# GAP-LAB-CUHK-SZ/RfDNet

Hardware: AMD Instinct MI355X
Metric: scenes/sec end-to-end reconstruction (ScanNet, 64^3 MISE) (higher is better)
Workload: dtype f32 (point ops, MLPs); f16x3 split MFMA with f32 accumulate (decoder, fp32-class)

## Files before the change

### include/rfd_pointnet2.h

```cpp
#ifndef RFD_POINTNET2_H
#define RFD_POINTNET2_H

#ifdef __cplusplus
extern "C" {
#endif

int furthest_point_sampling_kernel_wrapper(int b, int n, int m,
                                           const float *dataset, float *temp,
                                           int *idxs, void *stream);

int gather_points_kernel_wrapper(int b, int c, int n, int npoints,
                                 const float *points, const int *idx,
                                 float *out, void *stream);

int gather_points_grad_kernel_wrapper(int b, int c, int n, int npoints,
                                      const float *grad_out, const int *idx,
                                      float *grad_points, void *stream);

int query_ball_point_kernel_wrapper(int b, int n, int m, float radius,
                                    int nsample, const float *new_xyz,
                                    const float *xyz, int *idx, void *stream);

int group_points_kernel_wrapper(int b, int c, int n, int npoints, int nsample,
                                const float *points, const int *idx,
                                float *out, void *stream);

int group_points_grad_kernel_wrapper(int b, int c, int n, int npoints,
                                     int nsample, const float *grad_out,
                                     const int *idx, float *grad_points,
                                     void *stream);

int three_nn_kernel_wrapper(int b, int n, int m, const float *unknown,
                            const float *known, float *dist2, int *idx,
                            void *stream);

int three_interpolate_kernel_wrapper(int b, int c, int m, int n,
                                     const float *points, const int *idx,
                                     const float *weight, float *out,
                                     void *stream);

int three_interpolate_grad_kernel_wrapper(int b, int c, int n, int m,
                                          const float *grad_out,
                                          const int *idx, const float *weight,
                                          float *grad_points, void *stream);


int rfd_group_concat(int b, int c, int n, int m, int nsample, float radius,
                     int normalize, int use_xyz, const float *xyz,
                     const float *new_xyz, const float *features,
                     const int *idx, float *out, float *grouped_xyz_out,
                     void *stream);

int rfd_furthest_point_sampling_gather(int b, int n, int m,
                                       const float *dataset, float *temp,
                                       int *idxs, float *new_xyz,
                                       void *stream);

const char *rfd_last_error_string(void);
enum {
  RFD_STATUS_FPS_ABORT = 1,
  RFD_STATUS_DECODER_RANGE = 2,
  RFD_STATUS_GEMM_RANGE = 4
};
int rfd_device_status(void);
int rfd_stream_status(void *stream);
int rfd_stream_status_snapshot(void *stream, unsigned *host_word);
int rfd_release_stream(void *stream);
int rfd_fps_set_timeout_ms(int ms);
int rfd_fps_set_geometry(int points_per_thread);
int rfd_fps_test_phantom_units(int n);
int rfd_test_hold_cus(int leave_free_cus, const unsigned *release_flag, int max_ms, void *stream);
const char *rfd_build_arch(void);

int rfd_three_interpolate_cat(int b, int c, int cs, int m, int n, const float *points, const int *idx,
                              const float *dist2, const float *skip, float *out, void *stream);
int rfd_mlp_cols(int B, int N, int n_layers, const int *widths, const float *const *wt, const float *const *bias,
                 const int *relu, const float *x, float *y, void *stream);

int rfd_sa_fused(int b, int n, int m, int nsample, int c_feat, float radius, int normalize_xyz,
                 const float *xyz, const float *new_xyz, const float *features, const int *idx,
                 int c1, int c2, int c3, const float *w1, const float *b1, const float *w2,
                 const float *b2, const float *w3, const float *b3, float *out, void *stream);

#ifdef __cplusplus
}
#endif
#endif
```

### rfdnet_amd/_lib.py

```python
import ctypes as C
import os

_HERE = os.path.dirname(os.path.abspath(__file__))
LIB_PATH = os.environ.get("RFD_HIP_LIB") or os.path.join(_HERE, "lib", "librfd_hip.so")

_f = C.c_void_p
_i = C.c_int
_fl = C.c_float
_sz = C.c_size_t
_d = C.c_double

OPTIONAL = "optional"
ABI = {
    "furthest_point_sampling_kernel_wrapper": (_i, [_i, _i, _i, _f, _f, _f, _f]),
    "gather_points_kernel_wrapper": (_i, [_i, _i, _i, _i, _f, _f, _f, _f]),
    "gather_points_grad_kernel_wrapper": (_i, [_i, _i, _i, _i, _f, _f, _f, _f]),
    "query_ball_point_kernel_wrapper": (_i, [_i, _i, _i, _fl, _i, _f, _f, _f, _f]),
    "group_points_kernel_wrapper": (_i, [_i, _i, _i, _i, _i, _f, _f, _f, _f]),
    "group_points_grad_kernel_wrapper": (_i, [_i, _i, _i, _i, _i, _f, _f, _f, _f]),
    "three_nn_kernel_wrapper": (_i, [_i, _i, _i, _f, _f, _f, _f, _f]),
    "three_interpolate_kernel_wrapper": (_i, [_i, _i, _i, _i, _f, _f, _f, _f, _f]),
    "three_interpolate_grad_kernel_wrapper": (_i, [_i, _i, _i, _i, _f, _f, _f, _f, _f]),
    "rfd_group_concat": (_i, [_i, _i, _i, _i, _i, _fl, _i, _i, _f, _f, _f, _f, _f, _f, _f]),
    "rfd_furthest_point_sampling_gather": (_i, [_i, _i, _i, _f, _f, _f, _f, _f]),
    "rfd_chamfer_forward": (_i, [_i, _i, _f, _i, _f, _f, _f, _f, _f, _f]),
    "rfd_chamfer_backward": (_i, [_i, _i, _f, _i, _f, _f, _f, _f, _f, _f, _f, _f]),
    "rfd_sa_fused": (_i, [_i, _i, _i, _i, _i, _fl, _i, _f, _f, _f, _f, _i, _i, _i, _f, _f, _f, _f, _f, _f, _f, _f]),
    "rfd_occ_pack_weights": (_i, [_f, _f, C.POINTER(C.c_int), _i, _f, _f]),
    "rfd_occ_decode": (_i, [_i, _f, _f, _f, _f, _f, _f, _f, _fl, _f, _i, _f]),
    "rfd_occ_pack_weights_w8": (_i, [_f, _f, C.POINTER(C.c_int), _i, _f, _f]),
    "rfd_occ_decode_w8": (_i, [_i, _f, _f, _f, _f, _f, _f, _f, _fl, _f, _i, _f]),
    "rfd_occ_decode_scatter_w8": (_i, [_i, _f, _f, _f, _f, _f, _f, _f, _fl, _f, _f, _f, C.c_longlong, _i, _f]),
    "rfd_occ_chunk_range": (_i, [_i, _i, _i, C.POINTER(C.c_int), C.POINTER(C.c_int)]),
    "rfd_occ_chunk_range_capped": (_i, [_i, _i, _i, _i, C.POINTER(C.c_int), C.POINTER(C.c_int), C.POINTER(C.c_int)]),
    "rfd_occ_set_launch_shape": (_i, [_i, _i, _i]),
    "rfd_occ_set_tail_tiles": (_i, [_i]),
    "rfd_occ_normals_w8": (_i, [_i, _f, _f, _f, _i, _f, _f, C.POINTER(C.c_int), _f, _f, _f, _f, _f, _i, _f]),
    "rfd_refine_sample": (_i, [_i, _i, _f, _f, _f, _f, _f, _f, _f, _f, _f]),
    "rfd_refine_face_backward": (_i, [_i, _i, _f, _f, _f, _f, _f, _f, _f, _f, _fl, _f, _f]),
    "rfd_refine_vertex_step": (_i, [_i, _f, _f, _i, _f, _f, _f, _f, _f]),
    "rfd_refine_dirichlet": (_i, [_i, C.c_ulonglong, _i, _f, _f]),
    "rfd_fps_set_timeout_ms": (_i, [_i]),
    "rfd_fps_set_geometry": (_i, [_i]),
    "rfd_test_hold_cus": (_i, [_i, _f, _i, _f], OPTIONAL),
    "rfd_fps_test_phantom_units": (_i, [_i], OPTIONAL),
    "rfd_make_grid_points": (_i, [_i, _fl, _fl, _fl, _f, _i, _f]),
    "rfd_mise_init": (_i, [_i, _i, _i, _f, _f, _f]),
    "rfd_mise_count": (_i, [_i, _i, _i, _f, _f, _f]),
    "rfd_mise_collect": (_i, [_i, _i, _i, _f, _f, _f, _fl, _f, _f, _f]),
    "rfd_mise_scatter": (_i, [_i, _i, _i, _f, _f, _f, _f, _f, _f, _f]),
    "rfd_mise_subdivide": (_i, [_i, _i, _i, C.c_double, _f, _f, _f, _f]),
    "rfd_mise_subdivide_active": (_i, [_i, _i, _i, C.c_double, _f, _f, _f, _f, _f]),
    "rfd_mise_subdivide_dirty": (_i, [_i, _i, _i, C.c_double, _f, _f, _f, _f, C.c_longlong, _f, _f, _f, _f, _i, _f]),
    "rfd_mise_to_dense": (_i, [_i, _i, _i, _f, _f, _f]),
    "rfd_points_in_boxes": (_i, [_i, _i, _i, _i, _f, _f, _f, _f]),
    "rfd_nms3d": (_i, [_i, _i, C.c_double, _i, _i, _f, _f, _f, _f, _f, _f]),
    "rfd_gemm_pack_w": (_i, [_i, _i, _i, _f, _f, _f]),
    "rfd_gemm_f16x3": (_i, [_i, _i, _i, _f, _i, _f, _f, _i, _f, _f, _i, _f, _i, _i, _i, _i, _i, _f, _i, _f]),
    "rfd_mc_classify": (_i, [_i, _i, _fl, C.c_double, _f, _f, _f, _f, _f]),
    "rfd_mc_emit_affine": (_i, [_i, _i, _fl, C.c_double, _f, _f, _f, _f, _f, _f, _f, C.c_double, C.c_double, _f]),
    "rfd_mc_blocks": (_i, [_i]),
    "rfd_occ_fold_rows": (_i, [_i, _i, _i, _f, _f, _f, _f, _f, _f, _f, _i, _f, _f]),
    "rfd_rows3_rotate_z": (_i, [_i, _i, _f, _f, _f, _f]),
    "rfd_rows3_affine": (_i, [_i, _i, _f, _f, _f, _f]),
    "rfd_mlp_cols": (_i, [_i, _i, _i, _f, _f, _f, _f, _f, _f, _f]),
    "rfd_three_interpolate_cat": (_i, [_i, _i, _i, _i, _i, _f, _f, _f, _f, _f, _f]),
    "rfd_chain_pack_n": (_i, [_i, _i, _f, _f, _f, _i, _i, _i, _f, _f]),
    "rfd_chain_pool_n": (_i, [_i, _i, _i, _i, _i, _f, _i, _f, _f, _f, _f, _f, _i, _i, _i, _i, _i, _f, _f]),
    "rfd_head_pack": (_i, [_f, _f, _f, _i, _i, _i, _f, _f]),
    "rfd_head_scores": (_i, [_i, _i, _f, _i, _f, _f, _f, _f, _f, _f, _i, _i, _i, _i, _i, _f, _f]),
    "rfd_pos_embed": (_i, [_i, _i, _i, _f, _i, _f, _f, _i, _f, _f, _i, _f, _i, _i, _f]),
    "rfd_pos_embed_frag": (_i, [_i, _i, _i, _f, _i, _f, _f, _i, _f, _f, _i, _f, C.c_long, _i, _f]),
    "rfd_rows_to_frag": (_i, [_i, _i, _f, _i, _i, _i, _f, C.c_long, _f]),
    "rfd_frag_to_rows": (_i, [_i, _i, _f, C.c_long, _i, _f, _i, _f]),
    "rfd_gemm_f16x3_frag": (_i, [_i, _i, _i, _f, C.c_long, _f, _f, C.c_long, _f, _f, _i, _i, _i, _i, _f, _i, _f]),
    "rfd_box3d_iou": (_i, [_i, _i, _i, _f, _f, _f, _f, _f]),
    "rfd_ap_match": (_i, [_i, _i, _i, _i, _i, _f, _f, _f, _f, _f, _f, _f, _f]),
    "rfd_latent_prep": (_i, [_i, _i, _f, _f, _f, _f, _f, _f]),
    "rfd_latent_stage": (_i, [_i, _i, _i, _f, _f, _f, _f, _f, _f, _f, _f, _f]),
    "rfd_latent_head": (_i, [_i, _i, _f, _f, _f, _f, _f, _f, _f, _f, _f]),
    "rfd_bce_logits_rowsum": (_i, [_i, _i, _f, _i, _f, _i, _f, _f]),
    "rfd_voxel_iou": (_i, [_i, _i, _f, _i, _fl, _f, _f, _f, _f]),
    "rfd_vote_loss_partial": (_i, [_i, _i, _i, _i, _f, _f, _f, _f, _f, _f, _f]),
    "rfd_proposal_loss_partial": (_i, [_i, _i, _i, _i, _i, _i, _f, _f, _f, _f, _f, _f, _f, _f, C.POINTER(C.c_int), _f, _i, _f, _f,
                                       _f, _f, _f, _f, _f, _f, _f, _f, _i, _f, _f]),
    "rfd_detection_loss_finish": (_i, [_i, _i, _i, _f, _f, _f]),
    "rfd_mask_loss_partial": (_i, [_i, _i, _f, _f, _i, _f, _f, _f, _f]),
    "rfd_mask_loss_finish": (_i, [_i, _i, _fl, _f, _f, _f]),
    "rfd_fit_pose_run": (_i, [_i, _i, _i, _i, _i, _i, C.c_double, C.c_double, _f, _f, _f, _f, _f, _f, _f, _f, _f, _f, _f, _f,
                              _f, _f]),
    "rfd_raster_project": (_i, [_i, _i, _i, _f, _f, C.POINTER(C.c_double), C.c_double, _f, _f, _f, _f]),
    "rfd_raster_triangles": (_i, [_i, _i, _i, _i, _i, _i, _f, _f, _f, _f, _f, _f]),
    "rfd_raster_shade": (_i, [_i, _i, _i, _i, _i, _f, _f, _f, _f, _f, C.POINTER(C.c_double), _f, _f, _f, _f, _f]),
    "rfd_decimate_vertex_keys": (_i, [_i, _i, _i, _i, _f, _f, _f, _f, _f, _f]),
    "rfd_decimate_face_remap": (_i, [_i, _i, _i, _f, _f, _f, _f, _f, _f, _f, _f, _f]),
    "rfd_decimate_parity": (_i, [_i, _i, _i, _f, _f, _f, _f, _f, _f, _f]),
# ... 253 lines not shown
```

### rfdnet_amd/csrc/common.h

```cpp
#pragma once
#include <hip/hip_runtime.h>
#include <stdint.h>
#include <stdio.h>
#include <atomic>
#include "../../include/rfd_pointnet2.h"

#define RFD_API extern "C" __attribute__((visibility("default")))

void rfd_set_error(const char *where, hipError_t e);

#define RFD_CHECK(expr)                        \
  do {                                         \
    hipError_t _e = (expr);                    \
    if (_e != hipSuccess) {                    \
      rfd_set_error(#expr, _e);                \
      return (int)_e;                          \
    }                                          \
  } while (0)

#define RFD_CHECK_LAUNCH()                     \
  do {                                         \
    hipError_t _e = hipGetLastError();         \
    if (_e != hipSuccess) {                    \
      rfd_set_error(__func__, _e);             \
      return (int)_e;                          \
    }                                          \
  } while (0)

static inline int rfd_invalid(const char *msg) {
  const hipError_t e = hipErrorInvalidValue;
  rfd_set_error(msg, e);
  return (int)e;
}

constexpr int RFD_ZEROS_FLOATS = 16384;
constexpr int RFD_STATUS_SLOTS = 64;
constexpr int RFD_FPS_TIMEOUT_MS_DEFAULT = 500;
constexpr int FPS_MAX_WG = 256;
constexpr int FPS_REGION_HEAD = 8;
constexpr int FPS_REGION_GRANULES = FPS_REGION_HEAD + FPS_MAX_WG * 2 * 5;
constexpr int FPS_SHARED_RING = 16;
constexpr int FPS_REGIONS = RFD_STATUS_SLOTS + FPS_SHARED_RING;
constexpr int RFD_CLAIM_SLOTS = 1024;
struct RfdWorkspace {
  unsigned long long *fps_slots;
  unsigned *status;
  std::atomic<void *> status_owner[RFD_STATUS_SLOTS];
  float *zeros;
  unsigned *claim;
  std::atomic<unsigned> claim_seq;
  std::atomic<unsigned> ring_pos;
  int num_cu;
  int wall_clock_khz;
  std::atomic<int> fps_timeout_ms;
  std::atomic<int> fps_force_ppt;
  std::atomic<int> fps_test_phantom;
};
int rfd_get_workspace(RfdWorkspace **ws);
#define RFD_WORKSPACE(ws)                      \
  RfdWorkspace *ws;                            \
  do {                                         \
    int _rc = rfd_get_workspace(&ws);          \
    if (_rc) return _rc;                       \
  } while (0)
int rfd_status_slot(RfdWorkspace *ws, hipStream_t stream);
static inline unsigned *rfd_status_word(RfdWorkspace *ws, hipStream_t stream) {
  return ws->status + rfd_status_slot(ws, stream);
}
static inline unsigned *rfd_claim_pair(RfdWorkspace *ws, hipStream_t stream) {
  const int slot = rfd_status_slot(ws, stream);
  if (slot > 0) return ws->claim + 2 * slot;
  return ws->claim + 2 * (RFD_STATUS_SLOTS + ws->claim_seq.fetch_add(1, std::memory_order_relaxed) %
                                                 (RFD_CLAIM_SLOTS - RFD_STATUS_SLOTS));
}
static inline unsigned long long *rfd_fps_region(RfdWorkspace *ws, hipStream_t stream) {
  const int slot = rfd_status_slot(ws, stream);
  const unsigned r = slot > 0 ? (unsigned)slot
                              : RFD_STATUS_SLOTS + ws->ring_pos.fetch_add(1, std::memory_order_relaxed) % FPS_SHARED_RING;
  return ws->fps_slots + (size_t)r * FPS_REGION_GRANULES;
}

__device__ __forceinline__ float sumsq3(float a, float b, float c) {
  float t = b * b;
  t = __builtin_fmaf(a, a, t);
  t = __builtin_fmaf(c, c, t);
  return t;
}

__device__ __forceinline__ void atomic_max_float(float *p, float v) {
  if (v >= 0.f) atomicMax(reinterpret_cast<int *>(p), __float_as_int(v + 0.f));
  else atomicMin(reinterpret_cast<unsigned *>(p), __float_as_uint(v));
}

static inline int ceil_div(int a, int b) { return (a + b - 1) / b; }

static inline int ref_opt_n_threads(int work_size) {
  const int pow_2 = (int)(log((double)work_size) / log(2.0));
  int v = 1 << pow_2;
  if (v > 512) v = 512;
  if (v < 1) v = 1;
  return v;
}
```

### rfdnet_amd/csrc/runtime.hip

```cpp
#include "common.h"

#include <stdlib.h>

#include <mutex>
#include <string>

namespace {
thread_local std::string g_last_error;
std::mutex g_ws_mutex;
RfdWorkspace *g_ws[64] = {nullptr};
}

void rfd_set_error(const char *where, hipError_t e) {
  g_last_error = std::string(where) + ": " + hipGetErrorString(e);
}

int rfd_get_workspace(RfdWorkspace **out) {
  int dev = 0;
  RFD_CHECK(hipGetDevice(&dev));
  if (dev < 0 || dev >= 64) {
    rfd_set_error("rfd_get_workspace: device index", hipErrorInvalidDevice);
    return (int)hipErrorInvalidDevice;
  }
  std::lock_guard<std::mutex> lk(g_ws_mutex);
  if (!g_ws[dev]) {
    RfdWorkspace *w = new RfdWorkspace();
    RFD_CHECK(hipMalloc((void **)&w->fps_slots,
                        sizeof(unsigned long long) * (size_t)FPS_REGIONS * FPS_REGION_GRANULES));
    RFD_CHECK(hipMalloc((void **)&w->status, sizeof(unsigned) * RFD_STATUS_SLOTS));
    RFD_CHECK(hipMemset(w->status, 0, sizeof(unsigned) * RFD_STATUS_SLOTS));
    for (int i = 0; i < RFD_STATUS_SLOTS; ++i) w->status_owner[i].store(nullptr);
    RFD_CHECK(hipMalloc((void **)&w->zeros, sizeof(float) * RFD_ZEROS_FLOATS));
    RFD_CHECK(hipMemset(w->zeros, 0, sizeof(float) * RFD_ZEROS_FLOATS));
    RFD_CHECK(hipMalloc((void **)&w->claim, sizeof(unsigned) * 2 * RFD_CLAIM_SLOTS));
    RFD_CHECK(hipMemset(w->claim, 0, sizeof(unsigned) * 2 * RFD_CLAIM_SLOTS));
    w->claim_seq.store(0);
    w->ring_pos.store(0);
    w->num_cu = 0;
    (void)hipDeviceGetAttribute(&w->num_cu, hipDeviceAttributeMultiprocessorCount, dev);
    w->wall_clock_khz = 0;
    (void)hipDeviceGetAttribute(&w->wall_clock_khz, hipDeviceAttributeWallClockRate, dev);
    if (w->wall_clock_khz <= 0) w->wall_clock_khz = 100000;
    const char *to = getenv("RFD_FPS_TIMEOUT_MS");
    const int to_ms = to ? atoi(to) : 0;
    w->fps_timeout_ms.store(to_ms > 0 ? to_ms : RFD_FPS_TIMEOUT_MS_DEFAULT);
    w->fps_force_ppt.store(0);
    w->fps_test_phantom.store(0);
    g_ws[dev] = w;
  }
  *out = g_ws[dev];
  return 0;
}

RFD_API const char *rfd_last_error_string(void) { return g_last_error.c_str(); }

int rfd_status_slot(RfdWorkspace *ws, hipStream_t stream) {
  void *key = (void *)stream;
  if (!key) return 0;
  for (int i = 1; i < RFD_STATUS_SLOTS; ++i)
    if (ws->status_owner[i].load(std::memory_order_acquire) == key) return i;
  for (int i = 1; i < RFD_STATUS_SLOTS; ++i) {
    void *expected = nullptr;
    if (ws->status_owner[i].load(std::memory_order_acquire) == nullptr &&
        ws->status_owner[i].compare_exchange_strong(expected, key, std::memory_order_acq_rel))
      return i;
  }
  return 0;
}

RFD_API int rfd_device_status(void) {
  RfdWorkspace *ws;
  if (rfd_get_workspace(&ws)) return -1;
  unsigned v[RFD_STATUS_SLOTS];
  if (hipDeviceSynchronize() != hipSuccess) return -2;
  if (hipMemcpy(v, ws->status, sizeof(v), hipMemcpyDeviceToHost) != hipSuccess) return -3;
  unsigned all = 0;
  for (int i = 0; i < RFD_STATUS_SLOTS; ++i) all |= v[i];
  if (all) (void)hipMemset(ws->status, 0, sizeof(v));
  return (int)all;
}

RFD_API int rfd_stream_status(void *stream) {
  RfdWorkspace *ws;
  if (rfd_get_workspace(&ws)) return -1;
  unsigned *word = rfd_status_word(ws, (hipStream_t)stream);
  unsigned v = 0;
  if (hipMemcpyAsync(&v, word, sizeof(unsigned), hipMemcpyDeviceToHost, (hipStream_t)stream) != hipSuccess) return -3;
  if (hipStreamSynchronize((hipStream_t)stream) != hipSuccess) return -2;
  if (v) (void)hipMemsetAsync(word, 0, sizeof(unsigned), (hipStream_t)stream);
  return (int)v;
}

RFD_API int rfd_stream_status_snapshot(void *stream, unsigned *host_word) {
  RfdWorkspace *ws;
  if (rfd_get_workspace(&ws)) return -1;
  if (!host_word) return -3;
  unsigned *word = rfd_status_word(ws, (hipStream_t)stream);
  if (hipMemcpyAsync(host_word, word, sizeof(unsigned), hipMemcpyDeviceToHost, (hipStream_t)stream) != hipSuccess)
    return -3;
  if (hipMemsetAsync(word, 0, sizeof(unsigned), (hipStream_t)stream) != hipSuccess) return -3;
  return 0;
}

RFD_API int rfd_release_stream(void *stream) {
  RfdWorkspace *ws;
  if (rfd_get_workspace(&ws)) return -1;
  if (!stream) return 0;
  for (int i = 1; i < RFD_STATUS_SLOTS; ++i) {
    if (ws->status_owner[i].load(std::memory_order_acquire) != stream) continue;
    unsigned v = 0;
    if (hipStreamSynchronize((hipStream_t)stream) != hipSuccess) return -2;
    if (hipMemcpy(&v, ws->status + i, sizeof(unsigned), hipMemcpyDeviceToHost) != hipSuccess) return -3;
    if (v && hipMemset(ws->status + i, 0, sizeof(unsigned)) != hipSuccess) return -3;
    ws->status_owner[i].store(nullptr, std::memory_order_release);
    return (int)v;
  }
  return 0;
}

RFD_API int rfd_fps_set_timeout_ms(int ms) {
  RfdWorkspace *ws;
  if (rfd_get_workspace(&ws)) return -1;
  return ws->fps_timeout_ms.exchange(ms > 0 ? ms : RFD_FPS_TIMEOUT_MS_DEFAULT);
}

RFD_API int rfd_fps_set_geometry(int points_per_thread) {
  RfdWorkspace *ws;
  if (rfd_get_workspace(&ws)) return -1;
  switch (points_per_thread) {
    case 0: case 5: case 8: case 10: case 16: case 20: case 32: case 40: case 64: break;
    default: return -2;
  }
  return ws->fps_force_ppt.exchange(points_per_thread);
}

#ifndef RFD_NO_TEST_HOOKS
RFD_API int rfd_fps_test_phantom_units(int n) {
  RfdWorkspace *ws;
  if (rfd_get_workspace(&ws)) return -1;
  return ws->fps_test_phantom.exchange(n < 0 ? 0 : n > 8 ? 8 : n);
}
#endif

RFD_API const char *rfd_build_arch(void) { return "gfx950"; }
```

### rfdnet_amd/csrc/sampling.hip

```cpp
#include "common.h"

namespace {

constexpr int FPS_THREADS = 256;
constexpr int FPS_WAVES = FPS_THREADS / 64;
constexpr unsigned FPS_SLOW_POLLS = 256;

typedef unsigned long long u64;
typedef unsigned u32x4 __attribute__((ext_vector_type(4)));
typedef float f32x2 __attribute__((ext_vector_type(2)));

__device__ __forceinline__ unsigned wave_max_u32(unsigned v) {
  asm volatile(
      "s_nop 1\n\t"
      "v_max_u32_dpp %0, %0, %0 row_shr:1 row_mask:0xf bank_mask:0xf\n\t"
      "s_nop 1\n\t"
      "v_max_u32_dpp %0, %0, %0 row_shr:2 row_mask:0xf bank_mask:0xf\n\t"
      "s_nop 1\n\t"
      "v_max_u32_dpp %0, %0, %0 row_shr:4 row_mask:0xf bank_mask:0xf\n\t"
      "s_nop 1\n\t"
      "v_max_u32_dpp %0, %0, %0 row_shr:8 row_mask:0xf bank_mask:0xf\n\t"
      "s_nop 1\n\t"
      "v_max_u32_dpp %0, %0, %0 row_bcast:15 row_mask:0xa bank_mask:0xf\n\t"
      "s_nop 1\n\t"
      "v_max_u32_dpp %0, %0, %0 row_bcast:31 row_mask:0xc bank_mask:0xf\n\t"
      "s_nop 1"
      : "+v"(v));
  return (unsigned)__builtin_amdgcn_readlane((int)v, 63);
}

struct Cand {
  u64 key;
  int k;
  float x, y, z;
};

__device__ __forceinline__ Cand wave_select(const Cand &c) {
  const unsigned hi = (unsigned)(c.key >> 32), lo = (unsigned)c.key;
  const unsigned mh = wave_max_u32(hi);
  const unsigned ml = wave_max_u32(hi == mh ? lo : 0u);
  const u64 m = __ballot(hi == mh && lo == ml);
  const int src = __builtin_amdgcn_readfirstlane(__ffsll((long long)m) - 1);
  Cand r;
  r.key = ((u64)mh << 32) | ml;
  r.k = __builtin_amdgcn_readlane(c.k, src);
  r.x = __builtin_bit_cast(float, __builtin_amdgcn_readlane(__builtin_bit_cast(int, c.x), src));
  r.y = __builtin_bit_cast(float, __builtin_amdgcn_readlane(__builtin_bit_cast(int, c.y), src));
  r.z = __builtin_bit_cast(float, __builtin_amdgcn_readlane(__builtin_bit_cast(int, c.z), src));
  return r;
}

__device__ __forceinline__ unsigned fps_rank(int k, int bs_log2, int cpb) {
  const unsigned tid = (unsigned)k & ((1u << bs_log2) - 1u);
  const unsigned rev = bs_log2 ? (__brev(tid) >> (32 - bs_log2)) : 0u;
  return rev * (unsigned)cpb + ((unsigned)k >> bs_log2);
}

template <int PPT, bool MULTI>
__global__ __launch_bounds__(FPS_THREADS) void fps_kernel(
    int n, int m, int G, int Gw, int bs_log2, int cpb, const float *__restrict__ dataset,
    float *__restrict__ temp, int *__restrict__ idxs,
    float *__restrict__ new_xyz, u64 *region, unsigned *status, u64 timeout_ticks) {
  const int batch = blockIdx.x / G;
  const int g = blockIdx.x - batch * G;
  const int t = threadIdx.x;
  const int lane = t & 63, wave = t >> 6;
  dataset += (size_t)batch * n * 3;
  temp += (size_t)batch * n;
  idxs += (size_t)batch * m;
  if (new_xyz) new_xyz += (size_t)batch * m * 3;
  u64 *abort_word = region;
  u64 *slots = region + FPS_REGION_HEAD + (size_t)batch * Gw * 10;

  __shared__ int s_abort;
  __shared__ __attribute__((aligned(16))) u32x4 s_a[2][FPS_WAVES];
  __shared__ __attribute__((aligned(8))) f32x2 s_yz[2][FPS_WAVES];
  __shared__ __attribute__((aligned(16))) u32x4 s_win[2];
  __shared__ __attribute__((aligned(8))) f32x2 s_winyz[2];

  float px[PPT], py[PPT], pz[PPT], td[PPT];
  unsigned nrank[PPT];
  const int base = g * (PPT * FPS_THREADS) + t;
#pragma unroll
  for (int i = 0; i < PPT; ++i) {
    const int k = base + i * FPS_THREADS;
    const bool in = k < n;
    px[i] = in ? dataset[(size_t)k * 3 + 0] : 0.f;
    py[i] = in ? dataset[(size_t)k * 3 + 1] : 0.f;
    pz[i] = in ? dataset[(size_t)k * 3 + 2] : 0.f;
    const float mag = sumsq3(px[i], py[i], pz[i]);
    const bool skip = !in || ((double)mag <= 1e-3);
    nrank[i] = skip ? 0u : ~fps_rank(k, bs_log2, cpb);
    td[i] = skip ? 0.f : 1e10f;
  }
  const float p0x = dataset[0], p0y = dataset[1], p0z = dataset[2];

  float cx = p0x, cy = p0y, cz = p0z;
  if (g == 0 && t == 0) {
    idxs[0] = 0;
    if (new_xyz) { new_xyz[0] = p0x; new_xyz[1] = p0y; new_xyz[2] = p0z; }
  }
  if (t == 0) s_abort = 0;

  for (int j = 1; j < m; ++j) {
    const int par = j & 1;
    Cand c;
    c.key = 0; c.k = 0; c.x = p0x; c.y = p0y; c.z = p0z;
#pragma unroll
    for (int i = 0; i < PPT; ++i) {
// ... 148 lines not shown
  __shared__ unsigned char held[CU_LDS_BYTES];
  if (threadIdx.x == 0) {
    reinterpret_cast<volatile unsigned char *>(held)[CU_LDS_BYTES - 1] = 1;
    const u64 t0 = (u64)wall_clock64();
    while (__hip_atomic_load(release, __ATOMIC_RELAXED, __HIP_MEMORY_SCOPE_AGENT) == 0u &&
           (u64)wall_clock64() - t0 < max_ticks)
      __builtin_amdgcn_s_sleep(32);
  }
}
#endif

template <int PPT, bool MULTI>
int launch_fps(int nb, int n, int m, int G, int Gw, int bs_log2, int cpb,
               const float *dataset, float *temp, int *idxs, float *new_xyz,
               u64 *region, unsigned *status, u64 timeout_ticks, hipStream_t s) {
  hipLaunchKernelGGL((fps_kernel<PPT, MULTI>), dim3(nb * G), dim3(FPS_THREADS), 0, s, n,
                     m, G, Gw, bs_log2, cpb, dataset, temp, idxs, new_xyz, region,
                     status, timeout_ticks);
  RFD_CHECK_LAUNCH();
  return 0;
}

int fps_impl(int b, int n, int m, const float *dataset, float *temp, int *idxs,
             float *new_xyz, void *stream) {
  if (m <= 0 || b <= 0) return 0;
  if (n <= 0) return rfd_invalid("furthest_point_sampling: n <= 0");
  hipStream_t s = (hipStream_t)stream;
  RFD_WORKSPACE(ws);
  const int per_thread = ceil_div(n, FPS_THREADS);
  const int forced = ws->fps_force_ppt.load(std::memory_order_relaxed);
  int ppt, G;
  bool chosen = false;
  if (forced && per_thread > forced) {
    ppt = forced;
    G = ceil_div(n, FPS_THREADS * ppt);
    chosen = G > 1;
  }
  if (chosen) {
  } else if (per_thread <= 16) {
    G = 1;
    ppt = per_thread <= 1 ? 1 : per_thread <= 2 ? 2 : per_thread <= 4 ? 4 : per_thread <= 8 ? 8 : 16;
  } else {
    ppt = 10;
    G = ceil_div(n, FPS_THREADS * ppt);
    if (G > 64) { ppt = 16; G = ceil_div(n, FPS_THREADS * ppt); }
    if (G > 64) { ppt = 32; G = ceil_div(n, FPS_THREADS * ppt); }
    if (G > 64) { ppt = 64; G = ceil_div(n, FPS_THREADS * ppt); }
  }
  if (G > 64) return rfd_invalid("furthest_point_sampling: n > 1048576 unsupported");
  const int bs = ref_opt_n_threads(n);
  int bs_log2 = 0;
  while ((1 << bs_log2) < bs) ++bs_log2;
  const int cpb = ceil_div(n, bs);
  int Gw = G;
  if (G > 1) {
#ifndef RFD_NO_TEST_HOOKS
    const int phantom = ws->fps_test_phantom.exchange(0);
    Gw = G + phantom > 64 ? 64 : G + phantom;
#endif
  }
  const int batches_per_launch = G > 1 ? (FPS_MAX_WG / Gw) : b;
  const u64 timeout_ticks = (u64)ws->fps_timeout_ms.load(std::memory_order_relaxed) * (u64)ws->wall_clock_khz;
  unsigned *status = rfd_status_word(ws, s);
  for (int b0 = 0; b0 < b; b0 += batches_per_launch) {
    const int nb = (b - b0) < batches_per_launch ? (b - b0) : batches_per_launch;
    u64 *region = nullptr;
    if (G > 1) {
      region = rfd_fps_region(ws, s);
      RFD_CHECK(hipMemsetAsync(region, 0, sizeof(u64) * (FPS_REGION_HEAD + (size_t)nb * Gw * 10), s));
    }
    const float *ds = dataset + (size_t)b0 * n * 3;
    float *tp = temp + (size_t)b0 * n;
    int *ix = idxs + (size_t)b0 * m;
    float *nx = new_xyz ? new_xyz + (size_t)b0 * m * 3 : nullptr;
    int rc;
#define FPS_CASE(P, M) case P: rc = launch_fps<P, M>(nb, n, m, G, Gw, bs_log2, cpb, ds, tp, ix, nx, region, status, timeout_ticks, s); break;
    if (G > 1) {
      switch (ppt) {
        FPS_CASE(5, true) FPS_CASE(8, true) FPS_CASE(10, true) FPS_CASE(16, true) FPS_CASE(20, true) FPS_CASE(32, true)
        FPS_CASE(40, true) FPS_CASE(64, true)
        default: rc = (int)hipErrorInvalidValue;
      }
    } else {
      switch (ppt) {
        FPS_CASE(1, false) FPS_CASE(2, false) FPS_CASE(4, false) FPS_CASE(8, false) FPS_CASE(16, false)
        default: rc = (int)hipErrorInvalidValue;
      }
    }
#undef FPS_CASE
    if (rc) return rc;
  }
  return 0;
}

}

RFD_API int furthest_point_sampling_kernel_wrapper(int b, int n, int m,
                                                   const float *dataset,
                                                   float *temp, int *idxs,
                                                   void *stream) {
  return fps_impl(b, n, m, dataset, temp, idxs, nullptr, stream);
}

RFD_API int rfd_furthest_point_sampling_gather(int b, int n, int m,
                                               const float *dataset,
                                               float *temp, int *idxs,
// ... 45 lines not shown
```

Measured before the change: 19.82.

## Add spatially pruned furthest-point sampling using grid buckets and bounding-box culling

Adds a new FPS path that bins the points into a uniform grid of buckets sorted by cell, keeps a bounding box and per-bucket best candidate, and on each round only re-sweeps buckets whose box could be closer to the new centroid than their current max distance. This skips most of the distance updates a full sweep over all n points does each round. It runs as one 1024-thread block per batch and is chosen by default for 10k–40k points with m ≥ 1024. The cost is two extra preprocessing kernels, a per-stream scratch allocation, and less parallelism per scene than the existing multi-workgroup FPS.

```diff
diff --git a/include/rfd_pointnet2.h b/include/rfd_pointnet2.h
--- a/include/rfd_pointnet2.h
+++ b/include/rfd_pointnet2.h
@@ -68,6 +68,7 @@
 int rfd_release_stream(void *stream);
 int rfd_fps_set_timeout_ms(int ms);
 int rfd_fps_set_geometry(int points_per_thread);
+int rfd_fps_set_pruned(int mode);
 int rfd_fps_test_phantom_units(int n);
 int rfd_test_hold_cus(int leave_free_cus, const unsigned *release_flag, int max_ms, void *stream);
 const char *rfd_build_arch(void);
diff --git a/rfdnet_amd/_lib.py b/rfdnet_amd/_lib.py
--- a/rfdnet_amd/_lib.py
+++ b/rfdnet_amd/_lib.py
@@ -42,6 +42,7 @@
     "rfd_refine_dirichlet": (_i, [_i, C.c_ulonglong, _i, _f, _f]),
     "rfd_fps_set_timeout_ms": (_i, [_i]),
     "rfd_fps_set_geometry": (_i, [_i]),
+    "rfd_fps_set_pruned": (_i, [_i]),
     "rfd_test_hold_cus": (_i, [_i, _f, _i, _f], OPTIONAL),
     "rfd_fps_test_phantom_units": (_i, [_i], OPTIONAL),
     "rfd_make_grid_points": (_i, [_i, _fl, _fl, _fl, _f, _i, _f]),
diff --git a/rfdnet_amd/csrc/common.h b/rfdnet_amd/csrc/common.h
--- a/rfdnet_amd/csrc/common.h
+++ b/rfdnet_amd/csrc/common.h
@@ -55,8 +55,15 @@
   std::atomic<int> fps_timeout_ms;
   std::atomic<int> fps_force_ppt;
   std::atomic<int> fps_test_phantom;
+  std::atomic<int> fps_pruned_mode;
+  void *fps_scratch[FPS_REGIONS];
+  size_t fps_scratch_bytes[FPS_REGIONS];
 };
 int rfd_get_workspace(RfdWorkspace **ws);
+int rfd_fps_scratch(RfdWorkspace *ws, hipStream_t stream, size_t bytes, void **out);
+bool rfd_fps_pruned_wanted(RfdWorkspace *ws, int b, int n, int m);
+int rfd_fps_pruned(RfdWorkspace *ws, int b, int n, int m, int bs_log2, int cpb, const float *dataset, float *temp,
+                   int *idxs, float *new_xyz, hipStream_t stream);
 #define RFD_WORKSPACE(ws)                      \
   RfdWorkspace *ws;                            \
   do {                                         \
@@ -73,11 +80,13 @@
   return ws->claim + 2 * (RFD_STATUS_SLOTS + ws->claim_seq.fetch_add(1, std::memory_order_relaxed) %
                                                  (RFD_CLAIM_SLOTS - RFD_STATUS_SLOTS));
 }
+static inline unsigned rfd_fps_region_index(RfdWorkspace *ws, hipStream_t stream) {
+  const int slot = rfd_status_slot(ws, stream);
+  return slot > 0 ? (unsigned)slot
+                  : RFD_STATUS_SLOTS + ws->ring_pos.fetch_add(1, std::memory_order_relaxed) % FPS_SHARED_RING;
+}
 static inline unsigned long long *rfd_fps_region(RfdWorkspace *ws, hipStream_t stream) {
-  const int slot = rfd_status_slot(ws, stream);
-  const unsigned r = slot > 0 ? (unsigned)slot
-                              : RFD_STATUS_SLOTS + ws->ring_pos.fetch_add(1, std::memory_order_relaxed) % FPS_SHARED_RING;
-  return ws->fps_slots + (size_t)r * FPS_REGION_GRANULES;
+  return ws->fps_slots + (size_t)rfd_fps_region_index(ws, stream) * FPS_REGION_GRANULES;
 }
 
 __device__ __forceinline__ float sumsq3(float a, float b, float c) {
diff --git a/rfdnet_amd/csrc/fps_pruned.hip b/rfdnet_amd/csrc/fps_pruned.hip
--- /dev/null
+++ b/rfdnet_amd/csrc/fps_pruned.hip
@@ -0,0 +1,356 @@
+#include "common.h"
+#include "fps_wave.h"
+
+namespace {
+
+constexpr int PR_THREADS = 1024;
+constexpr int PR_WAVES = PR_THREADS / 64;
+constexpr int PR_MAX_CELLS = 512;
+constexpr int PR_MAX_BUCKETS = 1024;
+constexpr int PR_CAP_UNIT = 256;
+constexpr int PR_CAP_SPAN = 131072;
+constexpr int PR_UNROLL = 4;
+
+struct PrHeader {
+  float lo[3], inv[3];
+  int dim[3];
+  int nbuckets, nvalid, pad[5];
+  unsigned cursor[PR_MAX_CELLS];
+  uint2 range[PR_MAX_BUCKETS];
+};
+static_assert(sizeof(PrHeader) % 16 == 0, "the sorted points behind the header are read as float4");
+
+__host__ __device__ inline size_t pr_scene_bytes(int n) {
+  return sizeof(PrHeader) + ((size_t)n * (sizeof(float4) + sizeof(uint2)) + 15) / 16 * 16;
+}
+__device__ __forceinline__ float4 *pr_points(char *scene) { return reinterpret_cast<float4 *>(scene + sizeof(PrHeader)); }
+__device__ __forceinline__ uint2 *pr_meta(char *scene, int n) {
+  return reinterpret_cast<uint2 *>(scene + sizeof(PrHeader) + (size_t)n * sizeof(float4));
+}
+
+__device__ __forceinline__ bool pr_skipped(float x, float y, float z) {
+  return (double)sumsq3(x, y, z) <= 1e-3;
+}
+
+__device__ __forceinline__ int pr_axis(float f, int d) { return f >= 0.f ? (f < (float)d ? (int)f : d - 1) : 0; }
+__device__ __forceinline__ int pr_cell(const float *lo, const float *inv, const int *dim, float x, float y, float z) {
+  const int ix = pr_axis((x - lo[0]) * inv[0], dim[0]);
+  const int iy = pr_axis((y - lo[1]) * inv[1], dim[1]);
+  const int iz = pr_axis((z - lo[2]) * inv[2], dim[2]);
+  return (iz * dim[1] + iy) * dim[0] + ix;
+}
+
+__device__ __forceinline__ float wave_min_f32(float v) {
+#pragma unroll
+  for (int o = 32; o > 0; o >>= 1) v = fminf(v, __shfl_xor(v, o));
+  return v;
+}
+__device__ __forceinline__ float wave_max_f32(float v) {
+#pragma unroll
+  for (int o = 32; o > 0; o >>= 1) v = fmaxf(v, __shfl_xor(v, o));
+  return v;
+}
+
+__global__ __launch_bounds__(PR_THREADS) void fps_pruned_grid(int n, const float *__restrict__ dataset, char *scratch,
+                                                               size_t scene_bytes) {
+  const int t = threadIdx.x, lane = t & 63, wave = t >> 6;
+  dataset += (size_t)blockIdx.x * n * 3;
+  PrHeader *hdr = reinterpret_cast<PrHeader *>(scratch + (size_t)blockIdx.x * scene_bytes);
+  __shared__ float s_red[6][PR_WAVES];
+  __shared__ float s_lo[3], s_inv[3];
+  __shared__ int s_dim[3];
+  __shared__ unsigned s_cnt[PR_MAX_CELLS];
+  __shared__ unsigned s_pts[PR_MAX_CELLS], s_bkt[PR_MAX_CELLS];
+
+  float lo[3] = {INFINITY, INFINITY, INFINITY}, hi[3] = {-INFINITY, -INFINITY, -INFINITY};
+  for (int k = t; k < n; k += PR_THREADS) {
+    const float x = dataset[(size_t)k * 3], y = dataset[(size_t)k * 3 + 1], z = dataset[(size_t)k * 3 + 2];
+    if (pr_skipped(x, y, z)) continue;
+    lo[0] = fminf(lo[0], x); lo[1] = fminf(lo[1], y); lo[2] = fminf(lo[2], z);
+    hi[0] = fmaxf(hi[0], x); hi[1] = fmaxf(hi[1], y); hi[2] = fmaxf(hi[2], z);
+  }
+#pragma unroll
+  for (int a = 0; a < 3; ++a) {
+    const float l = wave_min_f32(lo[a]), h = wave_max_f32(hi[a]);
+    if (lane == 0) { s_red[a][wave] = l; s_red[3 + a][wave] = h; }
+  }
+  if (t < PR_MAX_CELLS) s_cnt[t] = 0;
+  __syncthreads();
+  if (t == 0) {
+    float ext[3];
+    for (int a = 0; a < 3; ++a) {
+      float l = s_red[a][0], h = s_red[3 + a][0];
+      for (int w = 1; w < PR_WAVES; ++w) { l = fminf(l, s_red[a][w]); h = fmaxf(h, s_red[3 + a][w]); }
+      s_lo[a] = l;
+      ext[a] = h - l;
+      s_dim[a] = 1;
+    }
+    const int target = n / 128 < PR_MAX_CELLS ? n / 128 : PR_MAX_CELLS;
+    for (int cells = 1; cells * 2 <= target; cells *= 2) {
+      int a = 0;
+      if (ext[1] / (float)s_dim[1] > ext[a] / (float)s_dim[a]) a = 1;
+      if (ext[2] / (float)s_dim[2] > ext[a] / (float)s_dim[a]) a = 2;
+      s_dim[a] *= 2;
+    }
+    for (int a = 0; a < 3; ++a) s_inv[a] = ext[a] > 0.f ? (float)s_dim[a] / ext[a] : 0.f;
+  }
+  __syncthreads();
+  for (int k = t; k < n; k += PR_THREADS) {
+    const float x = dataset[(size_t)k * 3], y = dataset[(size_t)k * 3 + 1], z = dataset[(size_t)k * 3 + 2];
+    if (pr_skipped(x, y, z)) continue;
+    atomicAdd(&s_cnt[pr_cell(s_lo, s_inv, s_dim, x, y, z)], 1u);
+  }
+  __syncthreads();
+  const unsigned cap = (unsigned)PR_CAP_UNIT * (unsigned)((n + PR_CAP_SPAN - 1) / PR_CAP_SPAN);
+  unsigned cnt = 0, vp = 0, vb = 0;
+  if (t < PR_MAX_CELLS) {
+    cnt = s_cnt[t];
+    vp = cnt;
+    vb = (cnt + cap - 1) / cap;
+    s_pts[t] = vp; s_bkt[t] = vb;
+  }
+  __syncthreads();
+  for (int o = 1; o < PR_MAX_CELLS; o <<= 1) {
+    unsigned ap = 0, ab = 0;
+    if (t < PR_MAX_CELLS && t >= o) { ap = s_pts[t - o]; ab = s_bkt[t - o]; }
+    __syncthreads();
+    if (t < PR_MAX_CELLS) { vp += ap; vb += ab; s_pts[t] = vp; s_bkt[t] = vb; }
+    __syncthreads();
+  }
+  if (t < PR_MAX_CELLS) {
+    const unsigned p0 = vp - cnt, nb = (cnt + cap - 1) / cap, b0 = vb - nb;
+    hdr->cursor[t] = p0;
+    for (unsigned i = 0; i < nb && b0 + i < (unsigned)PR_MAX_BUCKETS; ++i) {
+      const unsigned s = p0 + i * cap, e = s + cap < p0 + cnt ? s + cap : p0 + cnt;
+      hdr->range[b0 + i] = make_uint2(s, e);
+    }
+  }
+  if (t == 0) {
+    for (int a = 0; a < 3; ++a) { hdr->lo[a] = s_lo[a]; hdr->inv[a] = s_inv[a]; hdr->dim[a] = s_dim[a]; }
+    const unsigned nb = s_bkt[PR_MAX_CELLS - 1];
+    hdr->nbuckets = (int)(nb < (unsigned)PR_MAX_BUCKETS ? nb : (unsigned)PR_MAX_BUCKETS);
+    hdr->nvalid = (int)s_pts[PR_MAX_CELLS - 1];
+  }
+}
+
+__global__ __launch_bounds__(256) void fps_pruned_scatter(int n, int bs_log2, int cpb, const float *__restrict__ dataset,
+                                                           float *__restrict__ temp, char *scratch, size_t scene_bytes) {
+  const int k = blockIdx.x * 256 + threadIdx.x;
+  if (k >= n) return;
+  dataset += (size_t)blockIdx.y * n * 3;
+  temp += (size_t)blockIdx.y * n;
+  char *scene = scratch + (size_t)blockIdx.y * scene_bytes;
+  PrHeader *hdr = reinterpret_cast<PrHeader *>(scene);
+  const float x = dataset[(size_t)k * 3], y = dataset[(size_t)k * 3 + 1], z = dataset[(size_t)k * 3 + 2];
+  if (pr_skipped(x, y, z)) {
+    temp[k] = 1e10f;
+    return;
+  }
+  const unsigned pos = atomicAdd(&hdr->cursor[pr_cell(hdr->lo, hdr->inv, hdr->dim, x, y, z)], 1u);
+  if (pos >= (unsigned)n) return;
+  pr_points(scene)[pos] = make_float4(x, y, z, 1e10f);
+  pr_meta(scene, n)[pos] = make_uint2(~fps_rank(k, bs_log2, cpb), (unsigned)k);
+}
+
+struct PrOwn {
+  float lo[3], hi[3];
+  int beg, end;
+  u64 key;
+  float x, y, z;
+  int k;
+};
+
+struct PrChunks {
+  float4 p[PR_UNROLL];
+  uint2 mt[PR_UNROLL];
+};
+__device__ __forceinline__ void pr_load(PrChunks &r, int i0, int end, int lane, const float4 *pts, const uint2 *meta) {
+#pragma unroll
+  for (int u = 0; u < PR_UNROLL; ++u) {
+    const int i = i0 + u * 64 + lane;
+    const bool in = i < end;
+    r.p[u] = in ? pts[i] : make_float4(0.f, 0.f, 0.f, 0.f);
+    r.mt[u] = in ? meta[i] : make_uint2(0u, 0u);
+  }
+}
+
+template <bool FIRST>
+__device__ __forceinline__ void pr_eval(const PrChunks &r, int i0, int end, int lane, float qx, float qy, float qz,
+                                        float4 *pts, Cand &c, float *lo, float *hi) {
+#pragma unroll
+  for (int u = 0; u < PR_UNROLL; ++u) {
+    const int i = i0 + u * 64 + lane;
+    const bool in = i < end;
+    const float4 p = r.p[u];
+    float d2 = p.w;
+    if constexpr (FIRST) {
+      if (in) {
+        lo[0] = fminf(lo[0], p.x); lo[1] = fminf(lo[1], p.y); lo[2] = fminf(lo[2], p.z);
+        hi[0] = fmaxf(hi[0], p.x); hi[1] = fmaxf(hi[1], p.y); hi[2] = fmaxf(hi[2], p.z);
+      }
+    } else {
+      const float d = sumsq3(p.x - qx, p.y - qy, p.z - qz);
+      d2 = fminf(d, p.w);
+      if (in && d < p.w) pts[i].w = d2;
+    }
+    const u64 key = in ? (((u64)__float_as_uint(d2) << 32) | r.mt[u].x) : 0ull;
+    const bool better = key > c.key;
+    c.key = better ? key : c.key;
+    c.k = better ? (int)r.mt[u].y : c.k;
+    c.x = better ? p.x : c.x;
+    c.y = better ? p.y : c.y;
+    c.z = better ? p.z : c.z;
+  }
+}
+
+template <bool FIRST>
+__device__ __forceinline__ void pr_sweep(u64 todo, PrOwn &own, int lane, float qx, float qy, float qz, float4 *pts,
+                                         const uint2 *meta) {
+  PrChunks nxt;
+  int L = -1, beg = 0, end = 0;
+  if (todo) {
+    L = __ffsll((long long)todo) - 1;
+    beg = __builtin_amdgcn_readlane(own.beg, L);
+    end = __builtin_amdgcn_readlane(own.end, L);
+    pr_load(nxt, beg, end, lane, pts, meta);
+  }
+  while (L >= 0) {
+    const PrChunks cur = nxt;
+    const int cl = L, cb = beg, ce = end;
+    todo &= todo - 1;
+    L = -1;
+    if (todo) {
+      L = __ffsll((long long)todo) - 1;
+      beg = __builtin_amdgcn_readlane(own.beg, L);
+      end = __builtin_amdgcn_readlane(own.end, L);
+      pr_load(nxt, beg, end, lane, pts, meta);
+    }
+    Cand c;
+    c.key = 0; c.k = 0; c.x = 0.f; c.y = 0.f; c.z = 0.f;
+    float lo[3] = {INFINITY, INFINITY, INFINITY}, hi[3] = {-INFINITY, -INFINITY, -INFINITY};
+    pr_eval<FIRST>(cur, cb, ce, lane, qx, qy, qz, pts, c, lo, hi);
+    for (int i0 = cb + 64 * PR_UNROLL; i0 < ce; i0 += 64 * PR_UNROLL) {
+      PrChunks more;
+      pr_load(more, i0, ce, lane, pts, meta);
+      pr_eval<FIRST>(more, i0, ce, lane, qx, qy, qz, pts, c, lo, hi);
+    }
+    const Cand w = wave_select(c);
+    const bool mine = lane == cl;
+    own.key = mine ? w.key : own.key;
+    own.k = mine ? w.k : own.k;
+    own.x = mine ? w.x : own.x;
+    own.y = mine ? w.y : own.y;
+    own.z = mine ? w.z : own.z;
+    if constexpr (FIRST) {
+#pragma unroll
+      for (int a = 0; a < 3; ++a) {
+        const float l = wave_min_f32(lo[a]), h = wave_max_f32(hi[a]);
+        own.lo[a] = mine ? l : own.lo[a];
+        own.hi[a] = mine ? h : own.hi[a];
+      }
+    }
+  }
+}
+
+__global__ __launch_bounds__(PR_THREADS) void fps_pruned_rounds(int n, int m, const float *__restrict__ dataset,
+                                                                 float *__restrict__ temp, int *__restrict__ idxs,
+                                                                 float *__restrict__ new_xyz, char *scratch,
+                                                                 size_t scene_bytes) {
+  const int t = threadIdx.x, lane = t & 63, wave = t >> 6;
+  dataset += (size_t)blockIdx.x * n * 3;
+  temp += (size_t)blockIdx.x * n;
+  idxs += (size_t)blockIdx.x * m;
+  if (new_xyz) new_xyz += (size_t)blockIdx.x * m * 3;
+  char *scene = scratch + (size_t)blockIdx.x * scene_bytes;
+  const PrHeader *hdr = reinterpret_cast<const PrHeader *>(scene);
+  float4 *pts = pr_points(scene);
+  const uint2 *meta = pr_meta(scene, n);
+
+  __shared__ __attribute__((aligned(16))) u32x4 s_a[2][PR_WAVES];
+  __shared__ __attribute__((aligned(8))) f32x2 s_yz[2][PR_WAVES];
+
+  const int nb = hdr->nbuckets < PR_MAX_BUCKETS ? hdr->nbuckets : PR_MAX_BUCKETS;
+  const int nvalid = hdr->nvalid < n ? hdr->nvalid : n;
+  const int bkt = lane * PR_WAVES + wave;
+  PrOwn own;
+  {
+    uint2 r = bkt < nb ? hdr->range[bkt] : make_uint2(0u, 0u);
+    if (r.y > (unsigned)nvalid) r.y = (unsigned)nvalid;
+    if (r.x > r.y) r.x = r.y;
+    own.beg = (int)r.x; own.end = (int)r.y;
+    own.key = 0; own.k = 0; own.x = own.y = own.z = 0.f;
+#pragma unroll
+    for (int a = 0; a < 3; ++a) { own.lo[a] = 0.f; own.hi[a] = 0.f; }
+  }
+  pr_sweep<true>(__ballot(own.end > own.beg), own, lane, 0.f, 0.f, 0.f, pts, meta);
+
+  const float p0x = dataset[0], p0y = dataset[1], p0z = dataset[2];
+  float cx = p0x, cy = p0y, cz = p0z;
+  if (t == 0) {
+    idxs[0] = 0;
+    if (new_xyz) { new_xyz[0] = p0x; new_xyz[1] = p0y; new_xyz[2] = p0z; }
+  }
+
+  for (int j = 1; j < m; ++j) {
+    const int par = j & 1;
+    const float gx = fmaxf(fmaxf(own.lo[0] - cx, 0.f), cx - own.hi[0]);
+    const float gy = fmaxf(fmaxf(own.lo[1] - cy, 0.f), cy - own.hi[1]);
+    const float gz = fmaxf(fmaxf(own.lo[2] - cz, 0.f), cz - own.hi[2]);
+    const bool dirty = sumsq3(gx, gy, gz) < __uint_as_float((unsigned)(own.key >> 32));
+    pr_sweep<false>(__ballot(dirty), own, lane, cx, cy, cz, pts, meta);
+    Cand c;
+    c.key = own.key; c.k = own.k; c.x = own.x; c.y = own.y; c.z = own.z;
+    const Cand w = wave_select(c);
+    if (lane == 0) {
+      s_a[par][wave] = u32x4{(unsigned)w.key, (unsigned)(w.key >> 32), (unsigned)w.k, __float_as_uint(w.x)};
+      s_yz[par][wave] = f32x2{w.y, w.z};
+    }
+    __syncthreads();
+    Cand o;
+    o.key = 0; o.k = 0; o.x = 0.f; o.y = 0.f; o.z = 0.f;
+    if (lane < PR_WAVES) {
+      const u32x4 a = s_a[par][lane];
+      const f32x2 yz = s_yz[par][lane];
+      o.key = ((u64)a.y << 32) | a.x; o.k = (int)a.z; o.x = __uint_as_float(a.w); o.y = yz.x; o.z = yz.y;
+    }
+    Cand b = wave_select(o);
+    if (b.key == 0ull) { b.k = 0; b.x = p0x; b.y = p0y; b.z = p0z; }
+    cx = b.x; cy = b.y; cz = b.z;
+    if (t == 0) {
+      idxs[j] = b.k;
+      if (new_xyz) { new_xyz[j * 3 + 0] = b.x; new_xyz[j * 3 + 1] = b.y; new_xyz[j * 3 + 2] = b.z; }
+    }
+  }
+  __syncthreads();
+  for (int i = t; i < nvalid; i += PR_THREADS) {
+    const unsigned k = meta[i].y;
+    if (k < (unsigned)n) temp[k] = pts[i].w;
+  }
+}
+
+}
+
+bool rfd_fps_pruned_wanted(RfdWorkspace *ws, int b, int n, int m) {
+  const int mode = ws->fps_pruned_mode.load(std::memory_order_relaxed);
+  if (mode) return mode > 0;
+  if (ws->fps_force_ppt.load(std::memory_order_relaxed) || ws->fps_test_phantom.load(std::memory_order_relaxed))
+    return false;
+  return n >= 10000 && n <= 40000 && m >= 1024 && (size_t)b * (size_t)n <= ((size_t)1 << 22);
+}
+
+int rfd_fps_pruned(RfdWorkspace *ws, int b, int n, int m, int bs_log2, int cpb, const float *dataset, float *temp,
+                   int *idxs, float *new_xyz, hipStream_t s) {
+  const size_t scene_bytes = pr_scene_bytes(n);
+  void *scratch = nullptr;
+  int rc = rfd_fps_scratch(ws, s, scene_bytes * (size_t)b, &scratch);
+  if (rc) return rc;
+  hipLaunchKernelGGL(fps_pruned_grid, dim3(b), dim3(PR_THREADS), 0, s, n, dataset, (char *)scratch, scene_bytes);
+  RFD_CHECK_LAUNCH();
+  hipLaunchKernelGGL(fps_pruned_scatter, dim3(ceil_div(n, 256), b), dim3(256), 0, s, n, bs_log2, cpb, dataset, temp,
+                     (char *)scratch, scene_bytes);
+  RFD_CHECK_LAUNCH();
+  hipLaunchKernelGGL(fps_pruned_rounds, dim3(b), dim3(PR_THREADS), 0, s, n, m, dataset, temp, idxs, new_xyz,
+                     (char *)scratch, scene_bytes);
+  RFD_CHECK_LAUNCH();
+  return 0;
+}
diff --git a/rfdnet_amd/csrc/fps_wave.h b/rfdnet_amd/csrc/fps_wave.h
--- /dev/null
+++ b/rfdnet_amd/csrc/fps_wave.h
@@ -0,0 +1,57 @@
+#pragma once
+#include "common.h"
+
+typedef unsigned long long u64;
+typedef unsigned u32x4 __attribute__((ext_vector_type(4)));
+typedef float f32x2 __attribute__((ext_vector_type(2)));
+
+__device__ __forceinline__ unsigned wave_max_u32(unsigned v) {
+  asm volatile(
+      "s_nop 1\n\t"
+      "v_max_u32_dpp %0, %0, %0 row_shr:1 row_mask:0xf bank_mask:0xf\n\t"
+      "s_nop 1\n\t"
+      "v_max_u32_dpp %0, %0, %0 row_shr:2 row_mask:0xf bank_mask:0xf\n\t"
+      "s_nop 1\n\t"
+      "v_max_u32_dpp %0, %0, %0 row_shr:4 row_mask:0xf bank_mask:0xf\n\t"
+      "s_nop 1\n\t"
+      "v_max_u32_dpp %0, %0, %0 row_shr:8 row_mask:0xf bank_mask:0xf\n\t"
+      "s_nop 1\n\t"
+      "v_max_u32_dpp %0, %0, %0 row_bcast:15 row_mask:0xa bank_mask:0xf\n\t"
+      "s_nop 1\n\t"
+      "v_max_u32_dpp %0, %0, %0 row_bcast:31 row_mask:0xc bank_mask:0xf\n\t"
+      "s_nop 1"
+      : "+v"(v));
+  return (unsigned)__builtin_amdgcn_readlane((int)v, 63);
+}
+
+struct Cand {
+  u64 key;
+  int k;
+  float x, y, z;
+};
+
+__device__ __forceinline__ u64 wave_max_key(u64 key, int &src) {
+  const unsigned hi = (unsigned)(key >> 32), lo = (unsigned)key;
+  const unsigned mh = wave_max_u32(hi);
+  const unsigned ml = wave_max_u32(hi == mh ? lo : 0u);
+  const u64 m = __ballot(hi == mh && lo == ml);
+  src = __builtin_amdgcn_readfirstlane(__ffsll((long long)m) - 1);
+  return ((u64)mh << 32) | ml;
+}
+
+__device__ __forceinline__ Cand wave_select(const Cand &c) {
+  int src;
+  Cand r;
+  r.key = wave_max_key(c.key, src);
+  r.k = __builtin_amdgcn_readlane(c.k, src);
+  r.x = __builtin_bit_cast(float, __builtin_amdgcn_readlane(__builtin_bit_cast(int, c.x), src));
+  r.y = __builtin_bit_cast(float, __builtin_amdgcn_readlane(__builtin_bit_cast(int, c.y), src));
+  r.z = __builtin_bit_cast(float, __builtin_amdgcn_readlane(__builtin_bit_cast(int, c.z), src));
+  return r;
+}
+
+__device__ __forceinline__ unsigned fps_rank(int k, int bs_log2, int cpb) {
+  const unsigned tid = (unsigned)k & ((1u << bs_log2) - 1u);
+  const unsigned rev = bs_log2 ? (__brev(tid) >> (32 - bs_log2)) : 0u;
+  return rev * (unsigned)cpb + ((unsigned)k >> bs_log2);
+}
diff --git a/rfdnet_amd/csrc/runtime.hip b/rfdnet_amd/csrc/runtime.hip
--- a/rfdnet_amd/csrc/runtime.hip
+++ b/rfdnet_amd/csrc/runtime.hip
@@ -46,6 +46,8 @@
     w->fps_timeout_ms.store(to_ms > 0 ? to_ms : RFD_FPS_TIMEOUT_MS_DEFAULT);
     w->fps_force_ppt.store(0);
     w->fps_test_phantom.store(0);
+    w->fps_pruned_mode.store(0);
+    for (int i = 0; i < FPS_REGIONS; ++i) { w->fps_scratch[i] = nullptr; w->fps_scratch_bytes[i] = 0; }
     g_ws[dev] = w;
   }
   *out = g_ws[dev];
@@ -134,6 +136,28 @@
   return ws->fps_force_ppt.exchange(points_per_thread);
 }
 
+RFD_API int rfd_fps_set_pruned(int mode) {
+  RfdWorkspace *ws;
+  if (rfd_get_workspace(&ws)) return -1;
+  if (mode < -1 || mode > 1) return -2;
+  return ws->fps_pruned_mode.exchange(mode);
+}
+
+int rfd_fps_scratch(RfdWorkspace *ws, hipStream_t stream, size_t bytes, void **out) {
+  const unsigned r = rfd_fps_region_index(ws, stream);
+  std::lock_guard<std::mutex> lk(g_ws_mutex);
+  if (ws->fps_scratch_bytes[r] < bytes) {
+    if (ws->fps_scratch[r]) RFD_CHECK(hipFree(ws->fps_scratch[r]));
+    ws->fps_scratch[r] = nullptr;
+    ws->fps_scratch_bytes[r] = 0;
+    const size_t want = bytes + bytes / 4;
+    RFD_CHECK(hipMalloc(&ws->fps_scratch[r], want));
+    ws->fps_scratch_bytes[r] = want;
+  }
+  *out = ws->fps_scratch[r];
+  return 0;
+}
+
 #ifndef RFD_NO_TEST_HOOKS
 RFD_API int rfd_fps_test_phantom_units(int n) {
   RfdWorkspace *ws;
diff --git a/rfdnet_amd/csrc/sampling.hip b/rfdnet_amd/csrc/sampling.hip
--- a/rfdnet_amd/csrc/sampling.hip
+++ b/rfdnet_amd/csrc/sampling.hip
@@ -1,4 +1,5 @@
 #include "common.h"
+#include "fps_wave.h"
 
 namespace {
 
@@ -6,55 +7,6 @@
 constexpr int FPS_WAVES = FPS_THREADS / 64;
 constexpr unsigned FPS_SLOW_POLLS = 256;
 
-typedef unsigned long long u64;
-typedef unsigned u32x4 __attribute__((ext_vector_type(4)));
-typedef float f32x2 __attribute__((ext_vector_type(2)));
-
-__device__ __forceinline__ unsigned wave_max_u32(unsigned v) {
-  asm volatile(
-      "s_nop 1\n\t"
-      "v_max_u32_dpp %0, %0, %0 row_shr:1 row_mask:0xf bank_mask:0xf\n\t"
-      "s_nop 1\n\t"
-      "v_max_u32_dpp %0, %0, %0 row_shr:2 row_mask:0xf bank_mask:0xf\n\t"
-      "s_nop 1\n\t"
-      "v_max_u32_dpp %0, %0, %0 row_shr:4 row_mask:0xf bank_mask:0xf\n\t"
-      "s_nop 1\n\t"
-      "v_max_u32_dpp %0, %0, %0 row_shr:8 row_mask:0xf bank_mask:0xf\n\t"
-      "s_nop 1\n\t"
-      "v_max_u32_dpp %0, %0, %0 row_bcast:15 row_mask:0xa bank_mask:0xf\n\t"
-      "s_nop 1\n\t"
-      "v_max_u32_dpp %0, %0, %0 row_bcast:31 row_mask:0xc bank_mask:0xf\n\t"
-      "s_nop 1"
-      : "+v"(v));
-  return (unsigned)__builtin_amdgcn_readlane((int)v, 63);
-}
-
-struct Cand {
-  u64 key;
-  int k;
-  float x, y, z;
-};
-
-__device__ __forceinline__ Cand wave_select(const Cand &c) {
-  const unsigned hi = (unsigned)(c.key >> 32), lo = (unsigned)c.key;
-  const unsigned mh = wave_max_u32(hi);
-  const unsigned ml = wave_max_u32(hi == mh ? lo : 0u);
-  const u64 m = __ballot(hi == mh && lo == ml);
-  const int src = __builtin_amdgcn_readfirstlane(__ffsll((long long)m) - 1);
-  Cand r;
-  r.key = ((u64)mh << 32) | ml;
-  r.k = __builtin_amdgcn_readlane(c.k, src);
-  r.x = __builtin_bit_cast(float, __builtin_amdgcn_readlane(__builtin_bit_cast(int, c.x), src));
-  r.y = __builtin_bit_cast(float, __builtin_amdgcn_readlane(__builtin_bit_cast(int, c.y), src));
-  r.z = __builtin_bit_cast(float, __builtin_amdgcn_readlane(__builtin_bit_cast(int, c.z), src));
-  return r;
-}
-
-__device__ __forceinline__ unsigned fps_rank(int k, int bs_log2, int cpb) {
-  const unsigned tid = (unsigned)k & ((1u << bs_log2) - 1u);
-  const unsigned rev = bs_log2 ? (__brev(tid) >> (32 - bs_log2)) : 0u;
-  return rev * (unsigned)cpb + ((unsigned)k >> bs_log2);
-}
 
 template <int PPT, bool MULTI>
 __global__ __launch_bounds__(FPS_THREADS) void fps_kernel(
@@ -309,6 +261,8 @@
   int bs_log2 = 0;
   while ((1 << bs_log2) < bs) ++bs_log2;
   const int cpb = ceil_div(n, bs);
+  if (rfd_fps_pruned_wanted(ws, b, n, m))
+    return rfd_fps_pruned(ws, b, n, m, bs_log2, cpb, dataset, temp, idxs, new_xyz, s);
   int Gw = G;
   if (G > 1) {
 #ifndef RFD_NO_TEST_HOOKS
```

New measurement: 19.74, median of 2. No clear change (-0.4%).
